# hihixuyang/LQR-Obstacles

Measured on AMD Instinct MI355X. Metric: agent-pair LQR-obstacle evals/sec, higher is better.
Workload: dtype f64

## Files before the change

lqr-obstacles_amd/csrc/lqro_device.hpp:

```cpp
#pragma once
#include <hip/hip_runtime.h>
#include <stdint.h>

namespace lqro {

constexpr int kWave = 64;

#define LQRO_ROW_BIG (1 << 20)

#define LQRO_ST_PAIRS 0
#define LQRO_ST_PLANES 1
#define LQRO_ST_INSIDE 2
#define LQRO_ST_HULLOK 3
#define LQRO_ST_HULLFAIL 4
#define LQRO_ST_BACKUP 5
#define LQRO_ST_NREACH 6
#define LQRO_ST_GTESTS 7
#define LQRO_ST_MERGED 8
#define LQRO_ST_RETRY 9
#define LQRO_ST_TIMEOUT 10
#define LQRO_ST_NFAIL 11
#define LQRO_ST_MWIN 12
#define LQRO_ST_NBUILD 13
#define LQRO_ST_FAILS 16
#define LQRO_ST_FAILMAX 64
#define LQRO_ST_MWINS (LQRO_ST_FAILS + LQRO_ST_FAILMAX)
#define LQRO_ST_SWORK (LQRO_ST_MWINS + LQRO_ST_FAILMAX)
#define LQRO_ST_BWORK (LQRO_ST_SWORK + 1)
#define LQRO_ST_BMAX (LQRO_ST_SWORK + 2)
#define LQRO_ST_WORDS (LQRO_ST_SWORK + 4)

enum : int {
  LQRO_HC_HULL = 0,
  LQRO_HC_HULL_NEXT = 1,
  LQRO_HC_RETRY = 2,
  LQRO_HC_RETRY_NEXT = 3,
  LQRO_HC_ROW = 4,
  LQRO_HC_UNUSED5 = 5,
  LQRO_HC_HOT = 6,
  LQRO_HC_HOT_NEXT = 7,
  LQRO_HC_UNUSED8 = 8,
  LQRO_HC_LP4 = 9,
  LQRO_HC_LP4_NEXT = 10,
  LQRO_HC_LHAND = 11,
  LQRO_HC_LHAND_NEXT = 12,
  LQRO_HC_LDONE = 13,
  LQRO_HC_UNUSED14 = 14,
  LQRO_HC_FACET0 = 15,
  LQRO_HC_WORDS = 16
};

enum : int {
  LQRO_H2_PREV = 0,
  LQRO_H2_HOT1 = 1,
  LQRO_H2_HOT1_NEXT = 2,
  LQRO_H2_HOT2_NEXT = 3,
  LQRO_H2_HOT2_DONE = 4,
  LQRO_H2_SPEC = 5,
  LQRO_H2_SPEC_NEXT = 6,
  LQRO_H2_UNUSED7 = 7,
  LQRO_H2_WORDS = 8
};

enum : int {
  LQRO_PROF_HULL = 0,
  LQRO_PROF_HJOBS = LQRO_PROF_HULL + 32,
  LQRO_PROF_PAIR = LQRO_PROF_HJOBS + 2 * 4096,
  LQRO_PROF_LFAIL = LQRO_PROF_PAIR + 16 + 16,
  LQRO_PROF_LJOBS = LQRO_PROF_LFAIL + 16,
  LQRO_PROF_QW1 = LQRO_PROF_LJOBS + 4 * 4096,
  LQRO_PROF_QLONG = LQRO_PROF_QW1 + 64,
  LQRO_PROF_WORDS = LQRO_PROF_QLONG + 24 * 1024,
  LQRO_PROF_HULL_WORDS = LQRO_PROF_LFAIL
};

__device__ __forceinline__ int opaque(int x) {
  asm volatile("" : "+v"(x));
  return x;
}

__device__ __forceinline__ double uniform(double v) {
  const long long b = __double_as_longlong(v);
  const int lo = __builtin_amdgcn_readfirstlane((int)b);
  const int hi = __builtin_amdgcn_readfirstlane((int)(b >> 32));
  return __longlong_as_double(((long long)hi << 32) | (unsigned)lo);
}

__device__ __forceinline__ void wave_lds_sync() {
  __builtin_amdgcn_fence(__ATOMIC_RELEASE, "workgroup");
  __builtin_amdgcn_wave_barrier();
  __builtin_amdgcn_fence(__ATOMIC_ACQUIRE, "workgroup");
}

template <int CTRL, int ROWS>
__device__ __forceinline__ int dpp_i(int old, int x) {
  return __builtin_amdgcn_update_dpp(old, x, CTRL, ROWS, 0xF, false);
}
template <int CTRL, int ROWS>
__device__ __forceinline__ double dpp_d(double old, double x) {
  const long long o = __double_as_longlong(old), v = __double_as_longlong(x);
  const int lo = dpp_i<CTRL, ROWS>((int)o, (int)v);
  const int hi = dpp_i<CTRL, ROWS>((int)(o >> 32), (int)(v >> 32));
  return __longlong_as_double(((long long)hi << 32) | (unsigned)lo);
}
__device__ __forceinline__ int wave_incl_scan(int x) {
  x += dpp_i<0x111, 0xF>(0, x);
  x += dpp_i<0x112, 0xF>(0, x);
  x += dpp_i<0x114, 0xF>(0, x);
  x += dpp_i<0x118, 0xF>(0, x);
  x += dpp_i<0x142, 0xA>(0, x);
  x += dpp_i<0x143, 0xC>(0, x);
  return x;
}

__device__ __forceinline__ uint64_t mix64(uint64_t z) {
  z += 0x9E3779B97F4A7C15ull;
  z = (z ^ (z >> 30)) * 0xBF58476D1CE4E5B9ull;
  z = (z ^ (z >> 27)) * 0x94D049BB133111EBull;
  return z ^ (z >> 31);
}

__device__ inline void inverse3(const double* q, double* out) {
  double m[9], inv[9];
  int rp[3] = {0, 1, 2}, cp[3] = {0, 1, 2};
#pragma unroll
  for (int i = 0; i < 9; ++i) { m[i] = q[i]; inv[i] = (i % 4 == 0) ? 1.0 : 0.0; }
#pragma unroll
  for (int k = 0; k < 3; ++k) {
    double best = 0.0; int br = k, bc = k;
#pragma unroll
    for (int i = k; i < 3; ++i)
#pragma unroll
      for (int j = k; j < 3; ++j) {
        double a = fabs(m[rp[i] * 3 + cp[j]]);
        if (a > best) { best = a; br = i; bc = j; }
      }
    int t = rp[k]; rp[k] = rp[br]; rp[br] = t;
    t = cp[k]; cp[k] = cp[bc]; cp[bc] = t;
#pragma unroll
    for (int i = k + 1; i < 3; ++i) {
      double f = m[rp[i] * 3 + cp[k]] / m[rp[k] * 3 + cp[k]];
#pragma unroll
      for (int j = k + 1; j < 3; ++j) m[rp[i] * 3 + cp[j]] -= f * m[rp[k] * 3 + cp[j]];
#pragma unroll
      for (int j = 0; j < k; ++j) inv[rp[i] * 3 + rp[j]] -= f * inv[rp[k] * 3 + rp[j]];
      inv[rp[i] * 3 + rp[k]] = -f;
    }
  }
#pragma unroll
  for (int k = 2; k >= 0; --k) {
    double qk = m[rp[k] * 3 + cp[k]];
#pragma unroll
    for (int j = 0; j < 3; ++j) inv[rp[k] * 3 + j] /= qk;
#pragma unroll
    for (int i = 0; i < k; ++i) {
// ... 57 lines not shown
```

lqr-obstacles_amd/csrc/lqro_qh_front.inc:

```
int simplex[4];
{
  int maxpoints[6];
  S.max_outside = 0.0;
  S.MAXabs_coord = 0.0;
  S.MAXwidth = -DBL_MAX;
  S.MAXsumcoord = 0.0;
  for (int k = 0; k < 3; k++) {
    int mn, mx;
    qh_extreme(W.Pr, n, k, false, lane, &mn);
    qh_extreme(W.Pr, n, k, true, lane, &mx);
    const double maxk = W.Pr[3 * (size_t)mx + k], mink = W.Pr[3 * (size_t)mn + k];
    const double maxcoord = fmax(maxk, -mink);
    const double temp = maxk - mink;
    if (temp > S.MAXwidth) S.MAXwidth = temp;
    if (maxcoord > S.MAXabs_coord) S.MAXabs_coord = maxcoord;
    S.MAXsumcoord += maxcoord;
    maxpoints[2 * k] = mn;
    maxpoints[2 * k + 1] = mx;
    S.NEARzero[k] = 80 * S.MAXsumcoord * DBL_EPSILON;
  }
  {
    double maxdistsum = sqrt(3.0) * S.MAXabs_coord;
    if (S.MAXsumcoord < maxdistsum) maxdistsum = S.MAXsumcoord;
    S.DISTround = DBL_EPSILON * (3 * maxdistsum * 1.01 + S.MAXabs_coord);
    const double MINdenom_1 = fmax(1.0 / DBL_MAX, DBL_MIN);
    S.MINdenom = MINdenom_1 * S.MAXabs_coord;
    S.MINdenom_2 = sqrt(MINdenom_1 * 3) * S.MAXabs_coord;
    S.MINvisible = 0.0 + 2 * S.DISTround;
    S.MAXcoplanar = S.MINvisible;
    S.MINoutside = 2 * S.MINvisible;
  }
  {
    double maxcoord = -DBL_MAX, mincoord = DBL_MAX;
    int minx = -1, maxx = -1;
    for (int i = 0; i < 6; i++) {
      const double c = W.Pr[3 * (size_t)maxpoints[i]];
      if (maxcoord < c) { maxcoord = c; maxx = maxpoints[i]; }
      if (mincoord > c) { mincoord = c; minx = maxpoints[i]; }
    }
    double maxdet = maxcoord - mincoord;
    int ns = 0;
    simplex[ns++] = minx;
    if (maxx != minx) simplex[ns++] = maxx;
    if (ns < 2) { S.status |= QHS_INPUT; QH_FRONT_FAIL; }
    for (int i = 2; i < 4; i++) {
      const double prevdet = maxdet;
      int maxpoint = -1, maxnearzero = 0, nearzero;
      maxdet = -1.0;
      for (int m = 0; m < 6; m++) {
        const int p = maxpoints[m];
        bool ins = false;
        for (int t = 0; t < i; t++) ins |= simplex[t] == p;
        if (!ins && p != maxpoint) {
          double det = fabs(qh_detsimplex(S, W.Pr, simplex, i, p, &nearzero));
          if (det > maxdet) { maxdet = det; maxpoint = p; maxnearzero = nearzero; }
        }
      }
      const double targetdet = prevdet * S.MAXwidth;
      const bool falsenarrow = maxdet > 0.0 && maxdet / targetdet < 1.0e-3;
      if (maxpoint < 0 || maxnearzero || falsenarrow) {
        double key = -1.0;
        int idx = 0x7fffffff;
        for (int q = lane; q < n; q += 64) {
          bool skip = false;
          for (int t = 0; t < 6; t++) skip |= maxpoints[t] == q;
          for (int t = 0; t < i; t++) skip |= simplex[t] == q;
          if (skip) continue;
          const double det = fabs(qh_detsimplex(S, W.Pr, simplex, i, q, &nearzero));
          if (det > key || (det == key && q < idx)) { key = det; idx = q; }
        }
        for (int off = 32; off >= 1; off >>= 1) {
          const double ok = __shfl_xor(key, off);
          const int oi = __shfl_xor(idx, off);
          if (ok > key || (ok == key && oi < idx)) { key = ok; idx = oi; }
        }
        if (idx != 0x7fffffff && key > maxdet) { maxdet = key; maxpoint = idx; }
      }
      if (maxpoint < 0) { S.status |= QHS_INPUT; QH_FRONT_FAIL; }
      simplex[i] = maxpoint;
    }
  }
}
```

lqr-obstacles_amd/csrc/lqro_qhull3.hpp:

```cpp
#pragma once
#include "lqro_qhull.hpp"
#include "lqro_qhull3_prof.hpp"
#include "lqro_lp.hpp"

namespace lqro {

#ifndef Q3_NEWCAP
#define Q3_NEWCAP 128
#endif
#ifndef Q3_VISCAP
#define Q3_VISCAP 192
#endif
#define Q3_MOVCAP 16
#define Q3_HZCAP 24
#define Q3_COPCAP 8
#define Q3_FSTK 512
#define Q3_ND (Q3_NEWCAP + Q3_MOVCAP)
#define Q3_WAVES 4
#define Q3_HR 4
#ifndef Q3_W0_SLEEP
#define Q3_W0_SLEEP 1
#endif
#ifndef Q3_W1_SLEEP
#define Q3_W1_SLEEP 1
// ... 1606 lines not shown
    L.sp_status = st;
    L.sp_apex[0] = apex[0]; L.sp_apex[1] = apex[1]; L.sp_apex[2] = apex[2];
  }
}

__device__ inline void q3_prescan(const Q3W& W, Q3L& L, int lane, unsigned short ep, unsigned ep2, Q3QC& Q) {
  Q.pc_from = -1;
  const int from = L.sp_pos, qt = Q.pc_end;
  if (!L.sp_ok || L.sp_facet < 0 || from < 0) return;
  auto marked = [&](int f) -> bool {
    return f < Q3_FL ? q3_lds(L.mark[f]) == ep : q3_glb(W.mark2[f]) == ep2;
  };
  Q.pc_pos = -1;
  for (int qh = from; qh < qt;) {
    if (qh >= Q.qcb + Q.qcn || qh < Q.qcb) {
      Q.qcb = qh;
      Q.qcn = min(64, qt - qh);
      if (lane < Q.qcn) {
        Q.qf = W.fq[qh + lane];
        Q.qk = W.fqk[qh + lane];
        const HullPt e = W.fqc[qh + lane];
        Q.qx = e.x; Q.qy = e.y; Q.qz = e.z; Q.qp = e.q;
      }
    }
    bool good = false;
    if (lane < Q.qcn && Q.qcb + lane >= qh && Q.qcb + lane < qt) {
      const int fa = q3_fa(W, L, Q.qf);
      const unsigned c = q3_cc(W, L, Q.qf);
      good = (fa & QF_LIVE) && !marked(Q.qf) && q3_key(W, L, Q.qf) == Q.qk && (c & 0xffffu) > 0;
    }
    const unsigned long long b = __ballot(good);
    if (b) {
      const int l = __ffsll((long long)b) - 1;
      Q.pc_pos = Q.qcb + l;
      Q.pc_f = __builtin_amdgcn_readlane(Q.qf, l);
      Q.pc_k = (unsigned)__builtin_amdgcn_readlane((int)Q.qk, l);
      Q.pc_p = __builtin_amdgcn_readlane(Q.qp, l);
      Q.pc_x = hl_rl(Q.qx, l); Q.pc_y = hl_rl(Q.qy, l); Q.pc_z = hl_rl(Q.qz, l);
      break;
    }
    qh = Q.qcb + Q.qcn;
  }
  Q.pc_from = from;
}

__device__ inline void q3_prefetch(const Q3W& W, Q3L& L, int lane, int p) {
  const int nvis = L.sp_hnvis;
  int np = 0;
  for (int c0 = 0; c0 < nvis; c0 += 64) {
    const int vi = c0 + lane;
    int cnt = 0;
    if (vi < nvis) {
      const int f = L.sp_visf[vi];
      cnt = (int)(q3_cc(W, L, f) & 0xffffu) - (vi == 0 ? 1 : 0);
      L.pf_vsoff[vi] = W.soff[f];
      L.pf_vscnt[vi] = cnt;
    }
    np += __builtin_amdgcn_readlane(q3_scan_add(cnt), 63);
  }
  hl_sync();
  if (lane < np) {
    int a = 0, base = 0;
    for (;;) {
      const int k = L.pf_vscnt[a];
      if (lane < base + k || a == nvis - 1) break;
      base += k;
      ++a;
    }
    const int q = W.sb[L.pf_vsoff[a] + lane - base];
    HullPt r;
    r.x = W.Pr[3 * (size_t)q]; r.y = W.Pr[3 * (size_t)q + 1]; r.z = W.Pr[3 * (size_t)q + 2];
    r.q = q;
    r.pad = 0;
    L.pf_pre[lane] = r;
    L.pf_prea[lane] = (unsigned char)a;
  }
  hl_sync();
  if (lane == 0) {
    L.pf_np = np;
    q3_st_rel(&L.pf_done, p);
  }
}

__device__ inline void q3_build(const Q3W& W, Q3S& S, Q3L& L, int n, int lane) {
  q3_prof_stamp(S.pf);
  const unsigned long long ltmask = (1ull << lane) - 1ull;
  S.status = 0;
  S.nalloc = 1;
  S.nfs = 0;
  S.sbtop = 0;
  S.nnew = S.nvis = S.nmov = S.nold = 0;
  S.findbestnew = S.notsharp = 0;
  S.hgen = 0;
  S.egen = 0;
  S.keyc = 1;
  S.key0_last = 0;
  S.qhead = S.qtail = 0;
  if (W.FC > 65535) {
    S.status |= QHS_CAPACITY | Q3_CAPBIT(QHS_CAP_FACETS);
    return;
  }
#define QH_FRONT_FAIL return
#include "lqro_qh_front.inc"
#undef QH_FRONT_FAIL
  const int pset[4] = {simplex[3], simplex[2], simplex[1], simplex[0]};
  int fs[4];
  {
    int top = 1, tops[4];
    for (int i = 0; i < 4; i++) {
      fs[i] = S.nalloc++;
      tops[i] = top;
      top ^= 1;
    }
    for (int k = 0; k < 3; k++) {
      double c = 0.0;
      for (int t = 0; t < 4; t++) c += W.Pr[3 * (size_t)pset[t] + k];
      S.interior[k] = c / 4;
    }
    int fv[4][3];
    for (int i = 0; i < 4; i++) {
      int m = 0;
      for (int t = 0; t < 4; t++)
        if (t != i) fv[i][m++] = pset[t];
    }
    int ls = 0;
    double q[4][4];
    bool fl[4];
    q3_plane(S, ls, W.Pr + 3 * (size_t)fv[0][0], W.Pr + 3 * (size_t)fv[0][1], W.Pr + 3 * (size_t)fv[0][2], tops[0],
             q[0], &fl[0]);
    if (q3_distq(q[0], S.interior) > S.DISTround)
      for (int i = 0; i < 4; i++) tops[i] ^= 1;
    bool anyflip = false;
    for (int i = 0; i < 4; i++) {
      q3_plane(S, ls, W.Pr + 3 * (size_t)fv[i][0], W.Pr + 3 * (size_t)fv[i][1], W.Pr + 3 * (size_t)fv[i][2],
               tops[i], q[i], &fl[i]);
      anyflip |= fl[i];
    }
    if (anyflip) ls |= QHS_FLIPPED;
    int nbs[4][3];
    for (int i = 0; i < 4; i++) {
      int m = 0;
      for (int t = 0; t < 4; t++)
        if (t != i) nbs[i][m++] = fs[t];
    }
    double minangle = DBL_MAX;
    for (int i = 0; i < 4; i++)
      for (int t = 0; t < 3; t++) {
        int j = 0;
        for (int u = 0; u < 4; u++)
          if (fs[u] == nbs[i][t]) j = u;
        double angle = 0.0;
        for (int k = 0; k < 3; k++) angle += q[i][k] * q[j][k];
        if (angle < minangle) minangle = angle;
      }
    if (minangle < -0.99999999) ls |= QHS_NARROW;
    S.status |= ls;
    hl_sync();
    if (lane == 0)
      for (int i = 0; i < 4; i++) {
        const int f = fs[i];
        q3_set_facet(W, L, f, q[i], nbs[i][0], nbs[i][1], nbs[i][2],
                     QF_LIVE | (tops[i] ? QF_TOP : 0) | (fl[i] ? QF_FLIPPED : 0));
        q3_set_key(W, L, f, S.keyc + i);
        q3_set_cc(W, L, f, 0u);
        Q3V& v = W.vv[f];
        for (int t = 0; t < 3; t++) {
          for (int k = 0; k < 3; k++) v.p[3 * t + k] = W.Pr[3 * (size_t)fv[i][t] + k];
          v.id[t] = fv[i][t];
        }
      }
    S.keyc += 4;
    hl_sync();
    int np = 0;
    for (int c = 0; c < n; c += 64) {
      const int qi = c + lane;
      const bool ok = qi < n && qi != simplex[0] && qi != simplex[1] && qi != simplex[2] && qi != simplex[3];
      const unsigned long long b = __ballot(ok);
      if (ok) W.pq[np + __popcll(b & ltmask)] = qi;
      np += __popcll(b);
    }
    hl_sync();
    const double distoutside = fmax(2 * S.MINoutside, S.max_outside);
    for (int i = 0; i < 4; i++) {
      const int f = fs[i];
      int cnt = 0;
      const int off = S.sbtop;
      double mx = 0.0, cx = 0.0, cy = 0.0, cz = 0.0;
      int champ = -1, w = 0;
      for (int c = 0; c < np; c += 64) {
        const int pos = c + lane;
        HullPt pt;
        pt.x = pt.y = pt.z = 0.0;
        pt.q = -1;
        pt.pad = 0;
        double d = -DBL_MAX;
        if (pos < np) {
          pt.q = W.pq[pos];
          pt.x = W.Pr[3 * (size_t)pt.q]; pt.y = W.Pr[3 * (size_t)pt.q + 1]; pt.z = W.Pr[3 * (size_t)pt.q + 2];
          const double p[3] = {pt.x, pt.y, pt.z};
          d = q3_distq(q[i], p);
        }
        const bool out = pos < np && d >= distoutside;
        const bool keep = pos < np && !out;
        const unsigned long long bk = __ballot(keep);
        hl_sync();
        if (keep) W.pq[w + __popcll(bk & ltmask)] = pt.q;
        w += __popcll(bk);
        const unsigned long long bo = __ballot(out);
        if (bo) {
          int wpos = -1, wr = 0;
          q3_place(bo, lane, ltmask, d, pt, off, W.SB, cnt, mx, champ, cx, cy, cz, wpos, wr);
          if (wpos >= 0) W.sb[wpos] = wr;
        }
        hl_sync();
      }
      if (cnt) {
        if (off + cnt > W.SB) { S.status |= QHS_CAPACITY | Q3_CAPBIT(QHS_CAP_SB); return; }
        if (lane == 0) {
          W.sb[off + cnt - 1] = champ;
          W.soff[f] = off;
          W.fdist[f] = mx;
          q3_set_cc(W, L, f, (unsigned)cnt | ((unsigned)champ << 16));
        }
        S.sbtop += cnt;
      }
      np = w;
      hl_sync();
    }
    if (np > 0) {
      S.nnew = 4;
      if (lane == 0)
        for (int i = 0; i < 4; i++) {
          L.nslot[i] = fs[i];
          for (int k = 0; k < 4; k++) L.npl[4 * i + k] = q[i][k];
          L.nflag[i] = q3_fa(W, L, fs[i]);
          L.nn1[i] = L.nn2[i] = 0;
        }
      S.nmov = 0;
      S.findbestnew = 1;
      hl_sync();
      int rg;
      double rd;
      HullPt rpt, pre;
      pre.x = pre.y = pre.z = 0.0;
      pre.q = -1;
      pre.pad = 0;
      q3_locate_seq(W, S, L, np, 0, true, lane, pre, 0, false, rg, rd, rpt);
      q3_emit_seq(W, S, L, np, 0, true, lane, rg, rd, rpt);
      S.findbestnew = 0;
      S.nnew = 0;
      S.nmov = 0;
      hl_sync();
    }
    if (S.status & (QHS_INPUT | QHS_TOPOLOGY | QHS_CAPACITY)) return;
    {
      int order[4] = {fs[0], fs[1], fs[2], fs[3]};
      unsigned kk[4];
      for (int i = 0; i < 4; i++) kk[i] = q3_key(W, L, order[i]);
      for (int a = 0; a < 4; a++)
        for (int b = a + 1; b < 4; b++)
          if (kk[b] < kk[a]) {
            const unsigned tk = kk[a]; kk[a] = kk[b]; kk[b] = tk;
            const int to = order[a]; order[a] = order[b]; order[b] = to;
          }
      int best = -1;
      double bd = -DBL_MAX;
      for (int i = 0; i < 4; i++) {
        const int f = order[i];
        if ((q3_cc(W, L, f) & 0xffffu) && W.fdist[f] > bd) { best = f; bd = W.fdist[f]; }
      }
      hl_sync();
      if (best >= 0) {
        q3_set_key(W, L, best, 0u);
        for (int i = 0; i < 4; i++)
          if (order[i] == best) {
            for (int t = i; t > 0; t--) { order[t] = order[t - 1]; kk[t] = kk[t - 1]; }
            order[0] = best;
            kk[0] = 0;
            break;
          }
      }
      int qt = 0;
      for (int i = 0; i < 4; i++)
        if (q3_cc(W, L, order[i]) & 0xffffu) {
          if (lane == 0) {
            W.fq[qt] = order[i];
            W.fqk[qt] = kk[i];
            HullPt r;
            r.x = r.y = r.z = 0.0; r.q = -1; r.pad = 0;
            W.fqc[qt] = r;
          }
          qt++;
        }
      S.qhead = 0;
      S.qtail = qt;
      hl_sync();
    }
  }
  Q3T(0);
  if (lane == 0) {
    L.c_dist[0] = S.MINvisible; L.c_dist[1] = S.MAXcoplanar; L.c_dist[2] = S.DISTround;
    L.c_dist[3] = S.MINdenom; L.c_dist[4] = S.MINdenom_2;
    for (int k = 0; k < 3; k++) { L.c_dist[5 + k] = S.NEARzero[k]; L.c_interior[k] = S.interior[k]; }
  }
  int phase = 0;
  int qcb = 0, qcn = 0;
  int qf = 0, qp = -1;
  unsigned qk = 0;
  double qx = 0.0, qy = 0.0, qz = 0.0;
  for (;;) {
    int facet = -1, furthest = -1;
// ... 625 lines not shown
      const double d = qsel_dist16(q, P, vrel, n16);
      const unsigned k = q3_key(W, L, f);
      if (d < best || (d == best && k < bkey)) {
        best = d; bkey = k; bf = f;
        bn[0] = n16[0]; bn[1] = n16[1]; bn[2] = n16[2];
      }
    }
  }
  for (int off = 32; off >= 1; off >>= 1) {
    const double ob = __shfl_xor(best, off);
    const unsigned ok = (unsigned)__shfl_xor((int)bkey, off);
    const int of = __shfl_xor(bf, off);
    const double o0 = __shfl_xor(bn[0], off), o1 = __shfl_xor(bn[1], off), o2 = __shfl_xor(bn[2], off);
    if (ob < best || (ob == best && ok < bkey)) { best = ob; bkey = ok; bf = of; bn[0] = o0; bn[1] = o1; bn[2] = o2; }
  }
  const bool ok = !fail && nfac > 0 && bf >= 0;
  const bool stale = ok && bkey == minkey;
  const bool merged = (S.status & (QHS_COPLANAR | QHS_NONCONVEX | QHS_FLIPPED | QHS_NARROW | QHS_SINGULAR)) != 0;
  const bool mwin = ok && merged && q3_merge_suspect(W, L, S, lane, vrel, best, head);
  int bv[3] = {0, 0, 0};
  if (ok)
    for (int t = 0; t < 3; t++) bv[t] = W.vv[bf].id[t];
  int go = 0;
  if (lane == 0)
    go = qsel_commit(A, slot, xi, ok, stale, merged, mwin, best, bn, nfac, S.status, bv, A.row_lp != 0);
  hl_sync();
  return __builtin_amdgcn_readfirstlane(go) != 0;
}

__device__ inline void q3_row_lp(const HullArgs& A, Q3L& L, int slot, int lane) {
  static_assert(sizeof(L.pl) >= 2 * LQRO_EARLY_LP_MAX_NPR * 32, "q3_row_lp: the planes must fit");
  const int lrow = slot / A.npr;
  const int i = A.row_begin + lrow * A.row_stride;
  float* planes = reinterpret_cast<float*>(L.pl);
  float* proj = planes + (size_t)A.npr * 8;
  __threadfence();
  const int m = lp_compact<8>(A.planes + (size_t)lrow * A.npr * 8, A.npr, planes, lane);
  const v3 pref = V3((float)A.lp_vgoal[3 * i], (float)A.lp_vgoal[3 * i + 1], (float)A.lp_vgoal[3 * i + 2]);
  v3 nv = V3(0.0f, 0.0f, 0.0f);
  const int fail = w_lp3<8>(planes, m, A.lp_vmax, pref, false, nv, lane);
  if (fail < m) w_lp4<8>(planes, m, fail, (float)A.lp_vmax, nv, proj, lane);
  if (lane == 0) {
    A.lp_newv[3 * i] = nv.x;
    A.lp_newv[3 * i + 1] = nv.y;
    A.lp_newv[3 * i + 2] = nv.z;
  }
  hl_sync();
}

#ifdef LQRO_QBIG_NOINLINE
__device__ __attribute__((noinline)) void q3_big_inline(const HullArgs& A, QhL& LB, int slot, unsigned long long tjob,
                                                        int wave) {
#else
__device__ inline void q3_big_inline(const HullArgs& A, QhL& LB, int slot, unsigned long long tjob, int wave) {
#endif
  const int lane = threadIdx.x & 63;
  const int HNP = A.H * A.NP;
  const QhW W = qh_worker(A.qscratch + (size_t)(A.block_base + blockIdx.x) * A.qstride, HNP);
  const HullJob J = hull_job(A, slot);
  const int n = hull_points(A, LB, J.Ti, J.Ni, J.xi, J.xj, J.vrel, W.Pr, W.Pf);
  if (wave == 0) qh_one_job(A, W, LB, J, n, slot, tjob, lane);
}

__device__ __forceinline__ void q3_body(const HullArgs& A, Q3L& L, QhL* LB = nullptr) {
  const int lane = threadIdx.x & 63;
  const int wave = __builtin_amdgcn_readfirstlane(threadIdx.x >> 6);
  const int HNP = A.H * A.NP;
  const Q3W W = q3_worker(A.qscratch + (size_t)(A.block_base + blockIdx.x) * A.qstride, HNP);
  for (;;) {
    const int slot = hull_take_job(A, L, false);
    if (slot < 0) break;
    const unsigned long long tjob = __builtin_amdgcn_s_memrealtime();
    const bool spec = A.spec_mark != nullptr && A.spec_mark[slot] >= 2;
    if (threadIdx.x == 0) {
      L.ph = 0; L.sp_done = 0; L.sp_gdone = 0; L.hctl = 0u; L.hbusy = 0; L.sp_hz = 0; L.pf_done = 0;
      L.ectl = 0u; L.edone = 0;
      L.qflags = A.qflags;
      q3_longprof_begin(L);
      L.big_slot = -1;
    }
    for (int q = threadIdx.x; q < Q3_FL / 2; q += blockDim.x) reinterpret_cast<unsigned*>(L.mark)[q] = 0u;
    const HullJob J = hull_job(A, slot);
    const int n = hull_points(A, L, J.Ti, J.Ni, J.xi, J.xj, J.vrel, W.Pr, W.Pf);
    bool lp_go = false;
    if (wave >= 2) {
      const Q3Col CH = q3_colh(W, wave, lane);
      int last = 0;
      long idle = 0;
      for (;;) {
        if (wave == 2) {
          const int hz = q3_ld_acq(&L.sp_hz);
          if (hz != last && hz > 0) {
            last = hz;
            q3_prefetch(W, L, lane, hz);
            idle = 0;
            continue;
          }
        }
        if (q3_help(W, L, lane, CH)) { idle = 0; continue; }
        if (q3_emit_help(W, L, lane)) { idle = 0; continue; }
        if (q3_ld_acq(&L.ph) < 0) break;
        if (++idle > (1l << 24)) break;
        __builtin_amdgcn_s_sleep(Q3_W2_SLEEP);
      }
    } else if (wave == 1) {
      unsigned* owner = qw_owner(A.qscratch + (size_t)(A.block_base + blockIdx.x) * A.qstride, A.qstride);
      if (*owner != QW_OWNER_Q3) {
        for (int q = lane; q < W.FC; q += 64) W.mark2[q] = 0u;
        if (lane == 0) { W.ctr[0] = 0u; *owner = QW_OWNER_Q3; }
      }
      unsigned ep2 = W.ctr[0];
      unsigned short ep = 0;
      const Q3Col CH = q3_colh(W, 1, lane);
      int last = 0;
      Q3QC Q;
      Q.qcb = 0; Q.qcn = 0; Q.qf = 0; Q.qp = -1; Q.qk = 0u; Q.qx = Q.qy = Q.qz = 0.0;
      Q.pc_from = -1; Q.pc_pos = -1; Q.pc_end = 0; Q.pc_f = 0; Q.pc_p = -1; Q.pc_k = 0u;
      Q.pc_x = Q.pc_y = Q.pc_z = 0.0;
      Q.one = 0; Q.rt = -1;
      for (int k = 0; k < 6; k++) Q.r[k] = 0.0;
      long idle = 0;
      Q3P P;
      for (int k = 0; k < 16; k++) P.t[k] = 0;
      for (;;) {
        const int p = q3_ld_acq(&L.ph);
        if (p != last) {
          if (p < 0) break;
          last = p;
          ++ep;
          ++ep2;
          Q3Cy t0;
          Q3Rt ts;
          q3_prof_spec_begin(L, P, t0, ts, lane);
          q3_spec(W, L, lane, ep, ep2, Q, P, p);
          hl_sync();
          q3_prof_spec_done(L, ts, lane);
          if (lane == 0) q3_st_rel_lds(&L.sp_done, p);
          if (lane == 0) q3_st_rel(&L.sp_gdone, p);
          if (L.qflags & 4) q3_prescan(W, L, lane, ep, ep2, Q);
          q3_prof_spec_end(L, P, t0, lane);
          idle = 0;
          continue;
        }
        {
          Q3Cy t0;
          q3_cy_now(t0);
          if (q3_help(W, L, lane, CH)) {
            q3_prof_w1_helped(P, t0);
            idle = 0;
            continue;
          }
        }
        if (q3_emit_help(W, L, lane)) { idle = 0; continue; }
        if (++idle > (1l << 24)) break;
        __builtin_amdgcn_s_sleep(Q3_W1_SLEEP);
      }
      q3_prof_w1_flush(A, P, lane);
      if (lane == 0) W.ctr[0] = ep2;
    } else {
    Q3S S;
    q3_prof_begin(S.pf);
    S.status = 0;
    S.nalloc = 1;
    S.nins = 0;
    if (L.fail || n < 4) S.status = QHS_INPUT;
    else q3_build(W, S, L, n, lane);
    hl_sync();
    if (lane == 0) q3_st_rel(&L.ph, -1);
    bool keep = true;
    if (spec) {
      int m = 0;
      if (lane == 0) {
        m = __hip_atomic_load(A.spec_mark + slot, __ATOMIC_ACQUIRE, __HIP_MEMORY_SCOPE_AGENT);
        for (long w = 0; m == 2 && w < (1l << 26); ++w) {
          __builtin_amdgcn_s_sleep(8);
          m = __hip_atomic_load(A.spec_mark + slot, __ATOMIC_ACQUIRE, __HIP_MEMORY_SCOPE_AGENT);
        }
        if (m == 2) {
          atomicAdd(&A.stats[LQRO_ST_TIMEOUT], 1ull);
          hull_fail_note(A.stats, slot);
        }
      }
      keep = __builtin_amdgcn_readfirstlane(m) == 3;
    }
    if (!keep) {
    } else if (S.status & QHS_CAPACITY) {
      if (lane == 0) {
        atomicAdd(&A.stats[LQRO_ST_RETRY], 1ull);
        if (S.status & QHS_TIMEOUT) atomicAdd(&A.stats[LQRO_ST_TIMEOUT], 1ull);
        if (LB) {
          L.big_slot = slot;
        } else {
          const int r = atomicAdd(A.rcount, 1);
          if (r < A.cap) A.rqueue[r] = slot;
        }
        hull_build_note(A, slot, 2, tjob, n, S.nins, S.nalloc - 1);
        q3_prof_retry(A, S.status, slot);
      }
      hl_sync();
    } else {
    q3_prof_stamp(S.pf);
    lp_go = q3_select(A, W, L, S, lane, J.xi, J.vrel, slot);
    if (lane == 0) q3_longprof_flush(A, hull_build_note(A, slot, 0, tjob, n, S.nins, S.nalloc - 1), S.pf, L);
    q3_prof_flush(A, S.pf, n, S.nalloc, lane);
    if (A.ext_nf && lane == 0) *A.ext_nf = S.status;
    if (A.ext_facets) {
      for (int f = 1 + lane; f < S.nalloc; f += 64) {
        if (!(q3_fa(W, L, f) & QF_LIVE)) continue;
        const unsigned k = q3_key(W, L, f);
        int rank = 0, nl = 0;
        for (int g = 1; g < S.nalloc; g++)
          if (q3_fa(W, L, g) & QF_LIVE) { nl++; rank += q3_key(W, L, g) < k; }
        if (rank < A.ext_max)
          for (int t = 0; t < 3; t++) A.ext_facets[3 * rank + t] = W.vv[f].id[t];
        if (rank == 0 && nl < A.ext_max) A.ext_facets[3 * nl] = -1;
      }
      hl_sync();
    }
    }
    }
#ifndef LQRO_QHULL_NO_INLINE_BIG
    if (LB) {
      __syncthreads();
      const int bs = L.big_slot;
      __syncthreads();
      if (bs >= 0) {
        q3_big_inline(A, *LB, bs, tjob, wave);
        __syncthreads();
      }
    }
#endif
    if (A.rowpend) {
      __syncthreads();
      if (wave == 0 && lp_go) q3_row_lp(A, L, slot, lane);
    }
  }
}

}
```

lqr-obstacles_amd/csrc/lqro_qhull3_prof.hpp:

```cpp
#pragma once
#include "lqro_hull_job.hpp"

namespace lqro {

#define Q3_PROF_RETRY (LQRO_PROF_PAIR + 16)
#ifdef LQRO_QHULL_PROFILE
#define Q3_CAPBIT(b) (b)
#else
#define Q3_CAPBIT(b) 0
#endif

struct Q3Prof {
#if defined(LQRO_QHULL_PROFILE) || defined(LQRO_QHULL_LONGPROF)
  unsigned long long tph[32];
  unsigned long long tq;
  unsigned long long tjob;
  unsigned long long tw, nw;
  unsigned long long tdl;
  unsigned long long tw1, nw1;
  unsigned long long tse, tsn;
  unsigned long long tfr, nsp;
  unsigned long long tfr2, trel;
  unsigned long long r_start, r_done, r_seen, r_gseen;
  unsigned long long tseen, tpre, npre, tstart;
  int prev1;
  unsigned long long tps[24], nps;
  unsigned long long lp_n, lp_pts, lp_t, lp_all, lp_tloc, lp_wait, lp_adopt, lp_tail, lp_tw;
  unsigned long long lp_own, lp_got, lp_hwait, lp_stop, lp_ev, lp_posts;
#endif
};

#if defined(LQRO_QHULL_PROFILE) && defined(LQRO_QHULL_PROF_LIGHT)
#define Q3T(k) do { const unsigned long long t_ = __builtin_amdgcn_s_memtime(); S.pf.tph[k] += t_ - S.pf.tq; S.pf.tq = t_; } while (0)
#elif defined(LQRO_QHULL_PROFILE)
#define Q3T(k) do { __builtin_amdgcn_s_waitcnt(0); const unsigned long long t_ = __builtin_amdgcn_s_memtime(); S.pf.tph[k] += t_ - S.pf.tq; S.pf.tq = t_; } while (0)
#else
#define Q3T(k) do {} while (0)
#endif
#define Q3_PROF_W1 LQRO_PROF_QW1
#define Q3_PROF_LONG LQRO_PROF_QLONG
struct Q3P {
  unsigned long long tq2 = 0;
  unsigned long long t[16];
  unsigned long long tq;
};
#if defined(LQRO_QHULL_PROFILE) && defined(LQRO_QHULL_PROF_LIGHT)
#define W1T(k) do { const unsigned long long t_ = __builtin_amdgcn_s_memtime(); P.t[k] += t_ - P.tq; P.tq = t_; } while (0)
#elif defined(LQRO_QHULL_PROFILE)
#define W1T(k) do { __builtin_amdgcn_s_waitcnt(0); const unsigned long long t_ = __builtin_amdgcn_s_memtime(); P.t[k] += t_ - P.tq; P.tq = t_; } while (0)
#else
#define W1T(k) do {} while (0)
#endif
#ifdef LQRO_QHULL_PROFILE
#define Q3C(k, v) do { S.pf.tph[k] += (unsigned long long)(v); } while (0)
#define W1C(k, v) do { P.t[k] += (unsigned long long)(v); } while (0)
#else
#define Q3C(k, v) do {} while (0)
#define W1C(k, v) do {} while (0)
#endif

struct Q3Cy {
#ifdef LQRO_QHULL_PROFILE
  unsigned long long t;
#endif
};
struct Q3Rt {
#ifdef LQRO_QHULL_LONGPROF
  unsigned long long t;
#endif
};
__device__ __forceinline__ void q3_cy_now(Q3Cy& c) {
#ifdef LQRO_QHULL_PROFILE
  c.t = __builtin_amdgcn_s_memtime();
#endif
}
__device__ __forceinline__ void q3_rt_now(Q3Rt& r) {
#ifdef LQRO_QHULL_LONGPROF
  r.t = __builtin_amdgcn_s_memrealtime();
#endif
}

struct Q3WaitProf {
#ifdef LQRO_QHULL_PROFILE
  unsigned long long tf;
  int spins;
#endif
  __device__ __forceinline__ void first() {
#ifdef LQRO_QHULL_PROFILE
    tf = __builtin_amdgcn_s_memtime();
#endif
  }
  __device__ __forceinline__ void spin() {
#ifdef LQRO_QHULL_PROFILE
    ++spins;
#endif
  }
};

struct Q3InsProf {
#ifdef LQRO_QHULL_PROFILE
  unsigned long long snap[21];
  unsigned long long tins;
#endif
  Q3Cy tw;
  Q3WaitProf wp;
  Q3Rt ta, t0;
};

struct Q3ScanProf {
  Q3Rt t0, t1;
#ifdef LQRO_QHULL_LONGPROF
// ... 17 lines not shown
  F.trel = 0;
  F.r_start = F.r_done = F.r_seen = F.r_gseen = 0;
  F.tseen = F.tpre = F.npre = F.tstart = 0;
  F.prev1 = 0;
  for (int k = 0; k < 24; k++) F.tps[k] = 0;
  F.nps = 0;
  F.tjob = __builtin_amdgcn_s_memtime();
#endif
}

__device__ __forceinline__ void q3_prof_stamp(Q3Prof& F) {
#ifdef LQRO_QHULL_PROFILE
  F.tq = __builtin_amdgcn_s_memtime();
#endif
}

__device__ __forceinline__ void q3_prof_flush(const HullArgs& A, Q3Prof& F, int n, int nalloc, int lane) {
#ifdef LQRO_QHULL_PROFILE
  F.tph[10] = __builtin_amdgcn_s_memtime() - F.tq;
  F.tph[27] = __builtin_amdgcn_s_memtime() - F.tjob;
  F.tph[28] = (unsigned long long)n;
  if (A.prof && lane == 0) {
    for (int k = 0; k < 32; k++)
      if (k != 26 && k != 11) atomicAdd(&A.prof[k], F.tph[k]);
    atomicAdd(&A.prof[Q3_PROF_W1 + 9], F.tw);
    atomicAdd(&A.prof[Q3_PROF_W1 + 10], F.nw);
    for (int k = 0; k < 24; k++) atomicAdd(&A.prof[Q3_PROF_W1 + 16 + k], F.tps[k]);
    atomicAdd(&A.prof[Q3_PROF_W1 + 40], F.nps);
    atomicAdd(&A.prof[Q3_PROF_W1 + 41], F.tdl);
    atomicAdd(&A.prof[Q3_PROF_W1 + 42], F.tw1);
    atomicAdd(&A.prof[Q3_PROF_W1 + 43], F.nw1);
    atomicAdd(&A.prof[Q3_PROF_W1 + 44], F.tse);
    atomicAdd(&A.prof[Q3_PROF_W1 + 45], F.tsn);
    atomicAdd(&A.prof[Q3_PROF_W1 + 46], F.tfr);
    atomicAdd(&A.prof[Q3_PROF_W1 + 47], F.nsp);
    atomicAdd(&A.prof[Q3_PROF_W1 + 48], F.tfr2);
    atomicAdd(&A.prof[Q3_PROF_W1 + 49], F.trel);
    atomicAdd(&A.prof[Q3_PROF_W1 + 50], F.r_start);
    atomicAdd(&A.prof[Q3_PROF_W1 + 51], F.r_done);
    atomicAdd(&A.prof[Q3_PROF_W1 + 52], F.r_seen);
    atomicAdd(&A.prof[Q3_PROF_W1 + 53], F.r_gseen);
    atomicAdd(&A.prof[Q3_PROF_W1 + 54], F.tpre);
    atomicAdd(&A.prof[Q3_PROF_W1 + 55], F.npre);
    atomicAdd(&A.prof[Q3_PROF_W1 + 56], F.tstart);
    atomicMax(&A.prof[26], F.tph[27]);
    const unsigned long long j = atomicAdd(&A.prof[11], 1ull);
    if (j < 4096) {
      A.prof[32 + 2 * j] = F.tph[27];
      A.prof[33 + 2 * j] = F.tph[21] | ((unsigned long long)n << 20) | ((unsigned long long)nalloc << 40);
    }
  }
#endif
}

__device__ __forceinline__ void q3_prof_retry(const HullArgs& A, int status, int slot) {
#ifdef LQRO_QHULL_PROFILE
  if (A.prof) {
    const unsigned long long k = atomicAdd(&A.prof[Q3_PROF_RETRY], 1ull);
    atomicOr(&A.prof[Q3_PROF_RETRY + 1], (unsigned long long)status);
    if (k < 14) A.prof[Q3_PROF_RETRY + 2 + k] = (unsigned long long)slot | ((unsigned long long)status << 32);
  }
#endif
}

__device__ __forceinline__ void q3_prof_w1_flush(const HullArgs& A, const Q3P& P, int lane) {
#ifdef LQRO_QHULL_PROFILE
  if (A.prof && lane == 0)
    for (int k = 0; k < 16; k++) atomicAdd(&A.prof[Q3_PROF_W1 + k], P.t[k]);
#endif
}

template <class LT>
__device__ __forceinline__ void q3_longprof_begin(LT& L) {
#ifdef LQRO_QHULL_LONGPROF
  for (int k = 0; k < 12; k++) L.hprof[k] = 0ull;
  L.lp_pubr = L.lp_doner = 0ull;
#endif
}

template <class LT>
__device__ __forceinline__ void q3_longprof_flush(const HullArgs& A, int k, const Q3Prof& F, const LT& L) {
#ifdef LQRO_QHULL_LONGPROF
  if (A.prof && k >= 0 && k < 1024) {
    unsigned long long* r = A.prof + Q3_PROF_LONG + 24 * k;
    r[0] = F.lp_n; r[1] = F.lp_pts; r[2] = F.lp_t; r[3] = F.lp_all;
    r[4] = F.lp_tloc; r[5] = F.lp_wait; r[6] = F.lp_adopt - F.lp_wait; r[7] = F.lp_tail;
    r[8] = F.lp_own; r[9] = F.lp_got; r[10] = F.lp_hwait; r[11] = F.lp_stop; r[12] = F.lp_ev; r[13] = F.lp_posts;
    r[14] = L.hprof[0]; r[15] = L.hprof[1] | (L.hprof[2] << 32);
    for (int q = 3; q < 11; q++) r[13 + q] = L.hprof[q];
  }
#endif
}

#define Q3_PROF_LDS(r) (*(const __attribute__((address_space(3))) unsigned long long*)(&(r)))

template <class LT>
__device__ __forceinline__ void q3_lp_helped(LT& L, const Q3Rt& t0, const Q3Rt& t1) {
#ifdef LQRO_QHULL_LONGPROF
  const unsigned long long th2 = __builtin_amdgcn_s_memrealtime();
  atomicAdd(&L.hprof[0], 1ull);
  atomicAdd(&L.hprof[1], t1.t - t0.t);
  atomicAdd(&L.hprof[2], th2 - t0.t);
#endif
}

__device__ __forceinline__ void q3_lp_hwait(Q3Prof& F, const Q3Rt& tw0, bool waited) {
#ifdef LQRO_QHULL_LONGPROF
  if (waited) F.lp_hwait += __builtin_amdgcn_s_memrealtime() - tw0.t;
#endif
}
__device__ __forceinline__ void q3_lp_chunk(Q3Prof& F, bool mine) {
#ifdef LQRO_QHULL_LONGPROF
  if (mine) F.lp_own++; else F.lp_got++;
#endif
}
__device__ __forceinline__ void q3_lp_stopped(Q3Prof& F, const Q3Rt& ts0, bool help, bool ev) {
#ifdef LQRO_QHULL_LONGPROF
  if (help) {
    F.lp_stop += __builtin_amdgcn_s_memrealtime() - ts0.t;
    F.lp_posts++;
    if (ev) F.lp_ev++;
  }
#endif
}

__device__ __forceinline__ void q3_lp_scan_begin(Q3ScanProf& C) {
  q3_rt_now(C.t0);
#ifdef LQRO_QHULL_LONGPROF
  C.reloads = 0;
#endif
}
__device__ __forceinline__ void q3_lp_scan_reload(Q3ScanProf& C) {
#ifdef LQRO_QHULL_LONGPROF
  ++C.reloads;
#endif
}
template <class LT>
__device__ __forceinline__ void q3_lp_scan_end(LT& L, Q3ScanProf& C, int lane) {
  q3_rt_now(C.t1);
#ifdef LQRO_QHULL_LONGPROF
  if (lane == 0) { L.hprof[8] += (unsigned long long)C.reloads; L.hprof[9] += C.t1.t - C.t0.t; }
#endif
}
template <class LT>
__device__ __forceinline__ void q3_lp_horizon_end(LT& L, const Q3ScanProf& C, int lane) {
#ifdef LQRO_QHULL_LONGPROF
  if (lane == 0) L.hprof[10] += __builtin_amdgcn_s_memrealtime() - C.t1.t;
#endif
}

__device__ __forceinline__ void q3_prof_ins_begin(Q3Prof& F, Q3InsProf& I) {
#ifdef LQRO_QHULL_PROFILE
  for (int k = 0; k < 21; k++) I.snap[k] = F.tph[k];
#endif
  q3_rt_now(I.ta);
#ifdef LQRO_QHULL_LONGPROF
  F.lp_tail += F.lp_tw ? I.ta.t - F.lp_tw : 0ull;
#endif
}
__device__ __forceinline__ void q3_prof_wait_begin(Q3InsProf& I) {
  q3_cy_now(I.tw);
#ifdef LQRO_QHULL_PROFILE
  I.wp.spins = 0;
#endif
}
template <class LT>
__device__ __forceinline__ void q3_prof_wait_end(Q3Prof& F, LT& L, const Q3InsProf& I, int lane) {
#ifdef LQRO_QHULL_PROFILE
  if (F.prev1) { F.tfr += I.wp.tf - I.tw.t; F.nsp += (unsigned long long)I.wp.spins; }
#endif
#ifdef LQRO_QHULL_LONGPROF
  {
    const unsigned long long tn = __builtin_amdgcn_s_memrealtime();
    const unsigned long long de = Q3_PROF_LDS(L.lp_doner);
    if (tn - I.ta.t > 20 && tn > de && lane == 0) { L.hprof[6] += tn - de; L.hprof[7] += 1; }
  }
#endif
#ifdef LQRO_QHULL_PROFILE
  {
    const unsigned long long tn_ = __builtin_amdgcn_s_memtime();
    F.tw += tn_ - I.tw.t;
    F.nw += 1;
    if (tn_ - I.tw.t > 200) F.tdl += tn_ - L.done_t;
    F.tseen = tn_;
    if (F.prev1) {
      F.tw1 += tn_ - I.tw.t; F.nw1 += 1;
      F.tse += L.done_t - L.pub_t; F.tsn += tn_ - L.pub_t;
      F.tfr2 += L.done_t2 - L.pub_t;
      const unsigned long long nr_ = __builtin_amdgcn_s_memrealtime();
      F.r_start += L.start_r - L.pub_r; F.r_done += L.done_r - L.pub_r; F.r_seen += nr_ - L.pub_r;
    }
  }
#endif
#ifdef LQRO_QHULL_LONGPROF
  F.lp_wait += __builtin_amdgcn_s_memrealtime() - I.ta.t;
#endif
}
__device__ __forceinline__ void q3_prof_ins_chosen(const Q3Prof& F, Q3InsProf& I) {
#ifdef LQRO_QHULL_PROFILE
  I.tins = F.tq;
#endif
}
template <class LT>
__device__ __forceinline__ void q3_prof_publish(Q3Prof& F, LT& L, Q3InsProf& I, int lane) {
#ifdef LQRO_QHULL_PROFILE
  if (lane == 0) { L.pub_t = __builtin_amdgcn_s_memtime(); L.pub_r = __builtin_amdgcn_s_memrealtime(); }
  if (F.tseen) { F.tpre += __builtin_amdgcn_s_memtime() - F.tseen; F.npre += 1; }
#endif
  q3_rt_now(I.t0);
#ifdef LQRO_QHULL_LONGPROF
  F.lp_adopt += I.t0.t - I.ta.t;
  if (lane == 0) L.lp_pubr = I.t0.t;
#endif
}
template <class LT>
__device__ __forceinline__ void q3_prof_published(Q3Prof& F, const LT& L, int lane) {
#ifdef LQRO_QHULL_PROFILE
  if (lane == 0) F.trel += __builtin_amdgcn_s_memtime() - L.pub_t;
#endif
}
__device__ __forceinline__ void q3_lp_located(Q3Prof& F, const Q3InsProf& I, int np) {
#ifdef LQRO_QHULL_LONGPROF
  if (np > 64) F.lp_tloc += __builtin_amdgcn_s_memrealtime() - I.t0.t;
#endif
}
__device__ __forceinline__ void q3_lp_partitioned(Q3Prof& F, const Q3InsProf& I, int np) {
#ifdef LQRO_QHULL_LONGPROF
  const unsigned long long dt = __builtin_amdgcn_s_memrealtime() - I.t0.t;
  F.lp_all += dt;
  if (np > 64) { F.lp_n += 1; F.lp_pts += (unsigned long long)np; F.lp_t += dt; }
  F.lp_tw = I.t0.t + dt;
#endif
}
__device__ __forceinline__ void q3_prof_ins_end(Q3Prof& F, const Q3InsProf& I, int np) {
#ifdef LQRO_QHULL_PROFILE
  F.prev1 = np <= 64;
  if (np > 64) { F.tph[29] += F.tq - I.tins; F.tph[30] += 1; }
  else {
    for (int k = 0; k < 21; k++) F.tps[k] += F.tph[k] - I.snap[k];
    F.nps += 1;
  }
#endif
}

template <class LT>
__device__ __forceinline__ void q3_prof_spec_begin(LT& L, Q3P& P, Q3Cy& t0, Q3Rt& ts, int lane) {
  q3_cy_now(t0);
#ifdef LQRO_QHULL_PROFILE
  P.tq = t0.t;
  P.t[14] += t0.t - L.pub_t;
  if (P.tq2) P.t[15] += t0.t - P.tq2;
  if (lane == 0) L.start_r = __builtin_amdgcn_s_memrealtime();
#endif
  q3_rt_now(ts);
}
template <class LT>
__device__ __forceinline__ void q3_prof_spec_done(LT& L, const Q3Rt& ts, int lane) {
#ifdef LQRO_QHULL_LONGPROF
  if (lane == 0) {
    const unsigned long long te_ = __builtin_amdgcn_s_memrealtime();
    L.hprof[3] += 1; L.hprof[4] += ts.t - Q3_PROF_LDS(L.lp_pubr); L.hprof[5] += te_ - ts.t;
    L.lp_doner = te_;
  }
#endif
#ifdef LQRO_QHULL_PROFILE
  if (lane == 0) L.done_t = __builtin_amdgcn_s_memtime();
#endif
}
template <class LT>
__device__ __forceinline__ void q3_prof_spec_end(LT& L, Q3P& P, const Q3Cy& t0, int lane) {
#ifdef LQRO_QHULL_PROFILE
  if (lane == 0) { L.done_t2 = __builtin_amdgcn_s_memtime(); L.done_r = __builtin_amdgcn_s_memrealtime(); }
  P.tq2 = __builtin_amdgcn_s_memtime();
  P.t[0] += __builtin_amdgcn_s_memtime() - t0.t;
  P.t[7] += 1;
#endif
}
__device__ __forceinline__ void q3_prof_w1_helped(Q3P& P, const Q3Cy& t0) {
#ifdef LQRO_QHULL_PROFILE
  P.t[6] += __builtin_amdgcn_s_memtime() - t0.t;
  P.t[8] += 1;
#endif
}

}
```

Before: 59.75 million.

## Parallelize hull startup extremes and initial point partition across all waves

```diff
diff --git a/lqr-obstacles_amd/csrc/lqro_device.hpp b/lqr-obstacles_amd/csrc/lqro_device.hpp
--- a/lqr-obstacles_amd/csrc/lqro_device.hpp
+++ b/lqr-obstacles_amd/csrc/lqro_device.hpp
@@ -70,7 +70,7 @@
   LQRO_PROF_LJOBS = LQRO_PROF_LFAIL + 16,
   LQRO_PROF_QW1 = LQRO_PROF_LJOBS + 4 * 4096,
   LQRO_PROF_QLONG = LQRO_PROF_QW1 + 64,
-  LQRO_PROF_WORDS = LQRO_PROF_QLONG + 24 * 1024,
+  LQRO_PROF_WORDS = LQRO_PROF_QLONG + 32 * 1024,
   LQRO_PROF_HULL_WORDS = LQRO_PROF_LFAIL
 };
 
diff --git a/lqr-obstacles_amd/csrc/lqro_qh_front.inc b/lqr-obstacles_amd/csrc/lqro_qh_front.inc
--- a/lqr-obstacles_amd/csrc/lqro_qh_front.inc
+++ b/lqr-obstacles_amd/csrc/lqro_qh_front.inc
@@ -6,9 +6,13 @@
   S.MAXwidth = -DBL_MAX;
   S.MAXsumcoord = 0.0;
   for (int k = 0; k < 3; k++) {
+#ifdef QH_FRONT_MAXPOINTS
+    const int mn = QH_FRONT_MAXPOINTS[2 * k], mx = QH_FRONT_MAXPOINTS[2 * k + 1];
+#else
     int mn, mx;
     qh_extreme(W.Pr, n, k, false, lane, &mn);
     qh_extreme(W.Pr, n, k, true, lane, &mx);
+#endif
     const double maxk = W.Pr[3 * (size_t)mx + k], mink = W.Pr[3 * (size_t)mn + k];
     const double maxcoord = fmax(maxk, -mink);
     const double temp = maxk - mink;
diff --git a/lqr-obstacles_amd/csrc/lqro_qhull3.hpp b/lqr-obstacles_amd/csrc/lqro_qhull3.hpp
--- a/lqr-obstacles_amd/csrc/lqro_qhull3.hpp
+++ b/lqr-obstacles_amd/csrc/lqro_qhull3.hpp
@@ -1712,9 +1712,145 @@
   }
 }
 
-__device__ inline void q3_build(const Q3W& W, Q3S& S, Q3L& L, int n, int lane) {
+__device__ __forceinline__ void q3_extremes(const Q3W& W, Q3L& L, int n, int wave, int lane) {
+  const int step = (int)blockDim.x;
+  double key[6];
+  int idx[6];
+#pragma unroll
+  for (int j = 0; j < 6; j++) { key[j] = -DBL_MAX; idx[j] = 0x7fffffff; }
+  for (int q = 64 * wave + lane; q < n; q += step) {
+    double c[3];
+#pragma unroll
+    for (int k = 0; k < 3; k++) c[k] = q3_glb(W.Pr[3 * (size_t)q + k]);
+#pragma unroll
+    for (int j = 0; j < 6; j++) {
+      const double v = (j & 1) ? c[j >> 1] : -c[j >> 1];
+      if (v > key[j] || (v == key[j] && q < idx[j])) { key[j] = v; idx[j] = q; }
+    }
+  }
+#pragma unroll
+  for (int j = 0; j < 6; j++) {
+    for (int off = 32; off >= 1; off >>= 1) {
+      const double ok = __shfl_xor(key[j], off);
+      const int oi = __shfl_xor(idx[j], off);
+      if (ok > key[j] || (ok == key[j] && oi < idx[j])) { key[j] = ok; idx[j] = oi; }
+    }
+    if (lane == 0) { L.tr[6 * wave + j] = key[j]; L.tr[24 + 6 * wave + j] = (double)idx[j]; }
+  }
+  hl_bar();
+}
+
+__device__ __forceinline__ int q3_pa_dest(const double (*q)[4], const double* p, double distoutside, double& d) {
+  int dst = 4;
+  d = -DBL_MAX;
+#pragma unroll
+  for (int i = 3; i >= 0; i--) {
+    const double di = q3_distq(q[i], p);
+    if (di >= distoutside) { dst = i; d = di; }
+  }
+  return dst;
+}
+
+__device__ __forceinline__ bool q3_pa_count(const Q3W& W, Q3S& S, Q3L& L, int n, int lane, const int* simplex,
+                                            const double (*q)[4]) {
+  const double distoutside = fmax(2 * S.MINoutside, S.max_outside);
+  int cnt[4] = {0, 0, 0, 0};
+  double nx[3] = {0.0, 0.0, 0.0};
+  if (lane < n)
+#pragma unroll
+    for (int k = 0; k < 3; k++) nx[k] = q3_glb(W.Pr[3 * (size_t)lane + k]);
+  for (int c = 0; c < n; c += 64) {
+    const int qi = c + lane;
+    const double p[3] = {nx[0], nx[1], nx[2]};
+    if (qi + 64 < n)
+#pragma unroll
+      for (int k = 0; k < 3; k++) nx[k] = q3_glb(W.Pr[3 * (size_t)(qi + 64) + k]);
+    double d;
+    int dst = q3_pa_dest(q, p, distoutside, d);
+    if (qi >= n || qi == simplex[0] || qi == simplex[1] || qi == simplex[2] || qi == simplex[3]) dst = -1;
+#pragma unroll
+    for (int i = 0; i < 4; i++) cnt[i] += __popcll(__ballot(dst == i));
+  }
+  int off[4], top = S.sbtop;
+#pragma unroll
+  for (int i = 0; i < 4; i++) {
+    off[i] = top;
+    if (cnt[i]) {
+      if (top + cnt[i] > W.SB) { S.status |= QHS_CAPACITY | Q3_CAPBIT(QHS_CAP_SB); return false; }
+      top += cnt[i];
+    }
+  }
+  S.sbtop = top;
+  if (lane == 0) {
+    for (int i = 0; i < 4; i++) {
+      for (int k = 0; k < 4; k++) L.npl[4 * i + k] = q[i][k];
+      L.dcnt[i] = simplex[i];
+      L.doff[i] = off[i];
+    }
+    L.c_dist[0] = distoutside;
+  }
+  return true;
+}
+
+__device__ __forceinline__ int q3_pa_place(const Q3W& W, Q3L& L, int n, int wave, int lane) {
+  const unsigned long long ltmask = (1ull << lane) - 1ull;
+  const int nw = (int)(blockDim.x >> 6);
+  double q[4][4];
+  int simplex[4];
+#pragma unroll
+  for (int i = 0; i < 4; i++) {
+#pragma unroll
+    for (int k = 0; k < 4; k++) q[i][k] = L.npl[4 * i + k];
+    simplex[i] = L.dcnt[i];
+  }
+  const double distoutside = L.c_dist[0];
+  int w = 0;
+  for (int i = wave; i < 4; i += nw) {
+    const int off = L.doff[i], f = 1 + i;
+    int cnt = 0, champ = -1;
+    double mx = 0.0;
+    double nx[3] = {0.0, 0.0, 0.0};
+    if (lane < n)
+#pragma unroll
+      for (int k = 0; k < 3; k++) nx[k] = q3_glb(W.Pr[3 * (size_t)lane + k]);
+    for (int c = 0; c < n; c += 64) {
+      const int qi = c + lane;
+      const double p[3] = {nx[0], nx[1], nx[2]};
+      if (qi + 64 < n)
+#pragma unroll
+        for (int k = 0; k < 3; k++) nx[k] = q3_glb(W.Pr[3 * (size_t)(qi + 64) + k]);
+      double d;
+      int dst = q3_pa_dest(q, p, distoutside, d);
+      if (qi >= n || qi == simplex[0] || qi == simplex[1] || qi == simplex[2] || qi == simplex[3]) dst = -1;
+      if (i == 0) {
+        const unsigned long long bk = __ballot(dst == 4);
+        if (dst == 4) W.pq[w + __popcll(bk & ltmask)] = qi;
+        w += __popcll(bk);
+      }
+      const unsigned long long bo = __ballot(dst == i);
+      if (bo) {
+        HullPt pt;
+        pt.x = p[0]; pt.y = p[1]; pt.z = p[2];
+        pt.q = qi;
+        pt.pad = 0;
+        int wpos = -1, wr = 0;
+        double cx, cy, cz;
+        q3_place(bo, lane, ltmask, d, pt, off, W.SB, cnt, mx, champ, cx, cy, cz, wpos, wr);
+        if (wpos >= 0) W.sb[wpos] = wr;
+      }
+    }
+    if (cnt && lane == 0) {
+      W.sb[off + cnt - 1] = champ;
+      W.soff[f] = off;
+      W.fdist[f] = mx;
+      q3_set_cc(W, L, f, (unsigned)cnt | ((unsigned)champ << 16));
+    }
+  }
+  return w;
+}
+
+__device__ inline bool q3_start(const Q3W& W, Q3S& S, Q3L& L, int n, int lane, double (&q)[4][4]) {
   q3_prof_stamp(S.pf);
-  const unsigned long long ltmask = (1ull << lane) - 1ull;
   S.status = 0;
   S.nalloc = 1;
   S.nfs = 0;
@@ -1728,11 +1864,28 @@
   S.qhead = S.qtail = 0;
   if (W.FC > 65535) {
     S.status |= QHS_CAPACITY | Q3_CAPBIT(QHS_CAP_FACETS);
-    return;
-  }
-#define QH_FRONT_FAIL return
+    return false;
+  }
+  int maxpts[6];
+  {
+    const int nw = (int)(blockDim.x >> 6);
+    for (int j = 0; j < 6; j++) {
+      double key = L.tr[j];
+      int idx = (int)L.tr[24 + j];
+      for (int w = 1; w < nw; w++) {
+        const double ok = L.tr[6 * w + j];
+        const int oi = (int)L.tr[24 + 6 * w + j];
+        if (ok > key || (ok == key && oi < idx)) { key = ok; idx = oi; }
+      }
+      maxpts[j] = idx;
+    }
+  }
+#define QH_FRONT_FAIL return false
+#define QH_FRONT_MAXPOINTS maxpts
 #include "lqro_qh_front.inc"
+#undef QH_FRONT_MAXPOINTS
 #undef QH_FRONT_FAIL
+  q3_lp_start_front(S.pf);
   const int pset[4] = {simplex[3], simplex[2], simplex[1], simplex[0]};
   int fs[4];
   {
@@ -1754,7 +1907,6 @@
         if (t != i) fv[i][m++] = pset[t];
     }
     int ls = 0;
-    double q[4][4];
     bool fl[4];
     q3_plane(S, ls, W.Pr + 3 * (size_t)fv[0][0], W.Pr + 3 * (size_t)fv[0][1], W.Pr + 3 * (size_t)fv[0][2], tops[0],
              q[0], &fl[0]);
@@ -1801,62 +1953,16 @@
       }
     S.keyc += 4;
     hl_sync();
-    int np = 0;
-    for (int c = 0; c < n; c += 64) {
-      const int qi = c + lane;
-      const bool ok = qi < n && qi != simplex[0] && qi != simplex[1] && qi != simplex[2] && qi != simplex[3];
-      const unsigned long long b = __ballot(ok);
-      if (ok) W.pq[np + __popcll(b & ltmask)] = qi;
-      np += __popcll(b);
-    }
-    hl_sync();
-    const double distoutside = fmax(2 * S.MINoutside, S.max_outside);
-    for (int i = 0; i < 4; i++) {
-      const int f = fs[i];
-      int cnt = 0;
-      const int off = S.sbtop;
-      double mx = 0.0, cx = 0.0, cy = 0.0, cz = 0.0;
-      int champ = -1, w = 0;
-      for (int c = 0; c < np; c += 64) {
-        const int pos = c + lane;
-        HullPt pt;
-        pt.x = pt.y = pt.z = 0.0;
-        pt.q = -1;
-        pt.pad = 0;
-        double d = -DBL_MAX;
-        if (pos < np) {
-          pt.q = W.pq[pos];
-          pt.x = W.Pr[3 * (size_t)pt.q]; pt.y = W.Pr[3 * (size_t)pt.q + 1]; pt.z = W.Pr[3 * (size_t)pt.q + 2];
-          const double p[3] = {pt.x, pt.y, pt.z};
-          d = q3_distq(q[i], p);
-        }
-        const bool out = pos < np && d >= distoutside;
-        const bool keep = pos < np && !out;
-        const unsigned long long bk = __ballot(keep);
-        hl_sync();
-        if (keep) W.pq[w + __popcll(bk & ltmask)] = pt.q;
-        w += __popcll(bk);
-        const unsigned long long bo = __ballot(out);
-        if (bo) {
-          int wpos = -1, wr = 0;
-          q3_place(bo, lane, ltmask, d, pt, off, W.SB, cnt, mx, champ, cx, cy, cz, wpos, wr);
-          if (wpos >= 0) W.sb[wpos] = wr;
-        }
-        hl_sync();
-      }
-      if (cnt) {
-        if (off + cnt > W.SB) { S.status |= QHS_CAPACITY | Q3_CAPBIT(QHS_CAP_SB); return; }
-        if (lane == 0) {
-          W.sb[off + cnt - 1] = champ;
-          W.soff[f] = off;
-          W.fdist[f] = mx;
-          q3_set_cc(W, L, f, (unsigned)cnt | ((unsigned)champ << 16));
-        }
-        S.sbtop += cnt;
-      }
-      np = w;
-      hl_sync();
-    }
+    if (!q3_pa_count(W, S, L, n, lane, simplex, q)) return false;
+  }
+  return true;
+}
+
+__device__ inline void q3_build(const Q3W& W, Q3S& S, Q3L& L, int n, int lane, const double (&q)[4][4], int np) {
+  const unsigned long long ltmask = (1ull << lane) - 1ull;
+  const int fs[4] = {1, 2, 3, 4};
+  q3_lp_start_parted(S.pf);
+  {
     if (np > 0) {
       S.nnew = 4;
       if (lane == 0)
@@ -2648,6 +2754,27 @@
     for (int q = threadIdx.x; q < Q3_FL / 2; q += blockDim.x) reinterpret_cast<unsigned*>(L.mark)[q] = 0u;
     const HullJob J = hull_job(A, slot);
     const int n = hull_points(A, L, J.Ti, J.Ni, J.xi, J.xj, J.vrel, W.Pr, W.Pf);
+    Q3Rt tpts;
+    q3_rt_now(tpts);
+    q3_extremes(W, L, n, wave, lane);
+    Q3S S;
+    double q4[4][4];
+    if (wave == 0) {
+      q3_prof_begin(S.pf);
+      q3_lp_start_points(S.pf, tjob, tpts);
+      S.status = 0;
+      S.nalloc = 1;
+      S.nins = 0;
+      bool go = false;
+      if (L.fail || n < 4) S.status = QHS_INPUT;
+      else go = q3_start(W, S, L, n, lane, q4);
+      if (lane == 0) L.pcnt[0] = go ? 1 : 0;
+    }
+    hl_bar();
+    const bool started = L.pcnt[0] != 0;
+    int np0 = 0;
+    if (started) np0 = q3_pa_place(W, L, n, wave, lane);
+    hl_bar();
     bool lp_go = false;
     if (wave >= 2) {
       const Q3Col CH = q3_colh(W, wave, lane);
@@ -2724,13 +2851,7 @@
       q3_prof_w1_flush(A, P, lane);
       if (lane == 0) W.ctr[0] = ep2;
     } else {
-    Q3S S;
-    q3_prof_begin(S.pf);
-    S.status = 0;
-    S.nalloc = 1;
-    S.nins = 0;
-    if (L.fail || n < 4) S.status = QHS_INPUT;
-    else q3_build(W, S, L, n, lane);
+    if (started) q3_build(W, S, L, n, lane, q4, np0);
     hl_sync();
     if (lane == 0) q3_st_rel(&L.ph, -1);
     bool keep = true;
diff --git a/lqr-obstacles_amd/csrc/lqro_qhull3_prof.hpp b/lqr-obstacles_amd/csrc/lqro_qhull3_prof.hpp
--- a/lqr-obstacles_amd/csrc/lqro_qhull3_prof.hpp
+++ b/lqr-obstacles_amd/csrc/lqro_qhull3_prof.hpp
@@ -27,6 +27,7 @@
   unsigned long long tps[24], nps;
   unsigned long long lp_n, lp_pts, lp_t, lp_all, lp_tloc, lp_wait, lp_adopt, lp_tail, lp_tw;
   unsigned long long lp_own, lp_got, lp_hwait, lp_stop, lp_ev, lp_posts;
+  unsigned long long st_job, st_pts, st_front, st_part, st_pub;
 #endif
 };
 
@@ -210,12 +211,14 @@
 __device__ __forceinline__ void q3_longprof_flush(const HullArgs& A, int k, const Q3Prof& F, const LT& L) {
 #ifdef LQRO_QHULL_LONGPROF
   if (A.prof && k >= 0 && k < 1024) {
-    unsigned long long* r = A.prof + Q3_PROF_LONG + 24 * k;
+    unsigned long long* r = A.prof + Q3_PROF_LONG + 32 * k;
     r[0] = F.lp_n; r[1] = F.lp_pts; r[2] = F.lp_t; r[3] = F.lp_all;
     r[4] = F.lp_tloc; r[5] = F.lp_wait; r[6] = F.lp_adopt - F.lp_wait; r[7] = F.lp_tail;
     r[8] = F.lp_own; r[9] = F.lp_got; r[10] = F.lp_hwait; r[11] = F.lp_stop; r[12] = F.lp_ev; r[13] = F.lp_posts;
     r[14] = L.hprof[0]; r[15] = L.hprof[1] | (L.hprof[2] << 32);
     for (int q = 3; q < 11; q++) r[13 + q] = L.hprof[q];
+    r[24] = F.st_pts - F.st_job; r[25] = F.st_front - F.st_pts; r[26] = F.st_part - F.st_front;
+    r[27] = F.st_pub ? F.st_pub - F.st_part : 0ull;
   }
 #endif
 }
@@ -274,6 +277,24 @@
 __device__ __forceinline__ void q3_lp_horizon_end(LT& L, const Q3ScanProf& C, int lane) {
 #ifdef LQRO_QHULL_LONGPROF
   if (lane == 0) L.hprof[10] += __builtin_amdgcn_s_memrealtime() - C.t1.t;
+#endif
+}
+
+__device__ __forceinline__ void q3_lp_start_points(Q3Prof& F, unsigned long long tjob, const Q3Rt& tpts) {
+#ifdef LQRO_QHULL_LONGPROF
+  F.st_job = tjob;
+  F.st_pts = F.st_front = F.st_part = tpts.t;
+  F.st_pub = 0ull;
+#endif
+}
+__device__ __forceinline__ void q3_lp_start_front(Q3Prof& F) {
+#ifdef LQRO_QHULL_LONGPROF
+  F.st_front = F.st_part = __builtin_amdgcn_s_memrealtime();
+#endif
+}
+__device__ __forceinline__ void q3_lp_start_parted(Q3Prof& F) {
+#ifdef LQRO_QHULL_LONGPROF
+  F.st_part = __builtin_amdgcn_s_memrealtime();
 #endif
 }
 
@@ -339,6 +360,7 @@
 #ifdef LQRO_QHULL_LONGPROF
   F.lp_adopt += I.t0.t - I.ta.t;
   if (lane == 0) L.lp_pubr = I.t0.t;
+  if (!F.st_pub) F.st_pub = I.t0.t;
 #endif
 }
 template <class LT>
```

Result: no change. 59.71 million (-0.1%).
